# yinyunie/Pose2Room

Measured on AMD Instinct MI355X. Metric: P2RNet train-step samples/sec (T=1024,J=53,bs=32), higher is better.
Workload: dtype f32; 1 GPU; P2RNet full train step, bs=32/GPU, T=1024, J=53, seeds=512, proposals=128 (BASELINE configs[2]); input=P2RNet_dataloader over SyntheticPoseDataset, global_batch=32, frames=1024, parallelism=dp1

## Files before the change

### pose2room_amd/p2rnet/modules/stgcn.py

```python
import torch
import torch.nn as nn

from ..registers import MODULES
from .stgcn_layers import Graph, st_gcn_block
from .sub_modules import SingleConv


def _point_mlp(cin, width, cout):
    return nn.Sequential(SingleConv(cin, width, kernel_size=1, order='cbr', padding=0, ndim=1),
                         SingleConv(width, width, kernel_size=1, order='cbr', padding=0, ndim=1),
                         SingleConv(width, cout, kernel_size=1, order='c', padding=0, ndim=1))


@MODULES.register_module
class STGCN(nn.Module):
    def __init__(self, cfg, optim_spec=None):
        super().__init__()
        self.optim_spec = optim_spec

        self.graph = Graph(layout='virtualroom', strategy='spatial', max_hop=5)
        self.register_buffer('A', torch.tensor(self.graph.A, dtype=torch.float32, requires_grad=False))

        self.n_seeds = cfg.config['data']['num_seeds']
        self.origin_joint_id = cfg.dataset_config.origin_joint_id
        width, out_channels = 64, 256
        kernel_size = (3, self.A.size(0))
        self.knn = 20

        self.pos_embed = _point_mlp(3, 64, width)
        self.sk_feat = _point_mlp(3, 64, width)
        self.st_gcn_networks = nn.ModuleList(
            [st_gcn_block(width, 64, kernel_size, 1, residual=False)] +
            [st_gcn_block(64, 64, kernel_size, 1) for _ in range(5)])
        from ..gcn_op import GraphTables
        tables = GraphTables(self.graph.A)
        for i, blk in enumerate(self.st_gcn_networks):
            blk.gcn.tables = tables
            blk.chain_input = i > 0
        self.conv_joint = nn.Conv1d(cfg.dataset_config.joint_num * 64, out_channels, kernel_size=1)
        self.edge_importance = nn.ParameterList(
            [nn.Parameter(torch.ones(self.A.size())) for _ in self.st_gcn_networks])

        n_frames = cfg.config['data']['num_frames']
        if self.n_seeds >= n_frames:
            self.seed_inds = torch.round(torch.linspace(0, n_frames - 1, self.n_seeds)).long()
        else:
            self.seed_sampling = cfg.config['data']['seed_sampling']

    def _select_seeds(self, hip):
        n_batch, n_frames, _ = hip.shape
        device = hip.device
        if self.n_seeds >= n_frames:
            return self.seed_inds.repeat(n_batch, 1).to(device)
        if self.seed_sampling == 'random':
            inds = torch.argsort(torch.rand(size=(n_batch, n_frames)), dim=1)[:, :self.n_seeds]
            return torch.sort(inds, dim=1)[0].to(device)
        if self.seed_sampling == 'uniform':
            step = torch.norm(torch.diff(hip, dim=1), dim=2)
            cum = torch.cumsum(torch.cat([torch.zeros(size=(n_batch, 1), device=device), step], dim=1).double(),
                               dim=1).float()
            stride = cum[:, -1] / (self.n_seeds - 1)
            target = stride.unsqueeze(-1) * torch.arange(self.n_seeds, dtype=torch.float, device=device)
            if cum.is_cuda and cum.dtype == torch.float32 and n_frames <= 40000:
                from .. import seed_op
                return seed_op.nearest_prefix(cum, target)
            return torch.argmin(torch.abs(cum.unsqueeze(-1) - target.unsqueeze(1)), dim=1)
        raise NotImplementedError

    @staticmethod
    def _mlp(seq, x, inner, add_ct=None):
        from .. import bn_op, tconv_op, embed_op
        if embed_op.supported(seq, x, inner, add_ct):
            return embed_op.embed_mlp(seq, x, inner, add_ct)
        s0, s1, s2 = seq
        fused = (x.is_cuda and len(seq) == 3 and hasattr(s0, 'batchnorm') and hasattr(s1, 'batchnorm')
                 and not hasattr(s2, 'batchnorm') and tconv_op.supported_embed3(x, s0.conv)
                 and x.shape[2] % inner == 0 and inner <= 64)
        if fused:
            z0s = None
            if s0.batchnorm.training:
                z, z0s = tconv_op.embed3(x, s0.conv, want_stats=True)
            else:
                z = tconv_op.embed3(x, s0.conv)
            z = z.view(x.shape[0], 64, x.shape[2] // inner, inner)
            fused = tconv_op.supported_pointwise(z, s0.batchnorm, s1.conv) and \
                tconv_op.supported_pointwise(z, s1.batchnorm, s2.conv)
            if fused:
                if s1.batchnorm.training:
                    z, zs = tconv_op.bn_relu_tconv(z, s0.batchnorm, s1.conv, stats=z0s, want_stats=True)
                    z = tconv_op.bn_relu_tconv(z, s1.batchnorm, s2.conv, stats=zs, add_ct=add_ct)
                else:
                    z = tconv_op.bn_relu_tconv(z, s0.batchnorm, s1.conv)
                    z = tconv_op.bn_relu_tconv(z, s1.batchnorm, s2.conv, add_ct=add_ct)
                return z.view(x.shape[0], 64, x.shape[2])
        for stage in seq:
            if x.is_cuda and hasattr(stage, 'batchnorm') and hasattr(stage, 'ReLU') and \
                    bn_op.supported(x, stage.batchnorm):
                x = bn_op.fused_bn_act(stage.conv(x), stage.batchnorm, None, relu=True)
            else:
                x = stage(x)
        if add_ct is not None:
            x = (x.view(x.shape[0], x.shape[1], -1, inner) + add_ct.unsqueeze(-1)).view(x.shape)
        return x

    def embed(self, input_joints):
        n_batch, n_frames, n_joints, _ = input_joints.shape
        device = input_joints.device
        hip = input_joints[:, :, self.origin_joint_id]
        win = torch.arange(n_frames, device=device).unsqueeze(-1) + \
            torch.arange(-self.knn // 2, self.knn // 2, device=device).unsqueeze(0)
        win = win.clamp_(0, n_frames - 1)
        offs = hip[:, win] - hip.unsqueeze(2)
        pe = self._mlp(self.pos_embed, offs.reshape(n_batch, n_frames * self.knn, 3).transpose(1, 2).contiguous(), self.knn)
        from .. import seed_op
        pe = pe.view(n_batch, -1, n_frames, self.knn)
        fused = seed_op.short_rows_supported(pe)
        pe = seed_op.mean_last(pe) if fused else pe.mean(dim=3)
        rel = input_joints - input_joints[:, :, self.origin_joint_id:self.origin_joint_id + 1]
        sk = self._mlp(self.sk_feat, rel.reshape(n_batch, n_frames * n_joints, 3).transpose(1, 2).contiguous(), n_joints,
                       add_ct=pe)
        return sk.view(n_batch, -1, n_frames, n_joints)

    def forward(self, input_joints, end_points=None):
        end_points = {} if end_points is None else end_points
        n_batch, n_frames, n_joints, n_dim = input_joints.size()
        seed_inds = self._select_seeds(input_joints[:, :, self.origin_joint_id])

        x = self.embed(input_joints)
        blocks = self.st_gcn_networks
        tables = blocks[0].gcn.tables
        if tables is not None and tables.gen2 and all(b.chainable(x, self.A) for b in blocks):
            from ..gcn_op import prepare_chain
            for gcn, prep in zip(blocks, prepare_chain(blocks, self.A, self.edge_importance, tables, frames=x.shape[2])):
                x, _ = gcn(x, prep.Aeff, prepared=prep)
        else:
            for gcn, importance in zip(blocks, self.edge_importance):
                x, _ = gcn(x, self.A * importance)

        seed_skeleton = torch.gather(
            input_joints, 1, seed_inds[:, :, None, None].expand(n_batch, self.n_seeds, n_joints, n_dim))
        if self.n_seeds < n_frames:
            from .. import seed_op
            if seed_op.seed_rows_supported(x, seed_inds):
                rows = seed_op.seed_rows(x, seed_inds)
            else:
                rows = x.permute(0, 2, 1, 3)[torch.arange(n_batch, device=x.device)[:, None], seed_inds]
            seed_features = torch.nn.functional.linear(
                rows.reshape(n_batch, self.n_seeds, -1),
                self.conv_joint.weight.squeeze(-1), self.conv_joint.bias)
        else:
            x = x.transpose(2, 3).reshape(n_batch, -1, n_frames)
            seed_features = self.conv_joint(x).transpose(1, 2)
            seed_features = torch.gather(
                seed_features, 1, seed_inds.unsqueeze(-1).expand(n_batch, self.n_seeds, seed_features.size(-1)))
        end_points['seed_inds'] = seed_inds
        end_points['seed_skeleton'] = seed_skeleton[..., :3]
        end_points['seed_features'] = seed_features
        return end_points
```

### pose2room_amd/p2rnet/modules/stgcn_layers.py

```python
from collections import deque

import numpy as np
import torch
import torch.nn as nn

_VIRTUALROOM_BONES = [
    (0, 1), (1, 3), (3, 5), (5, 19), (0, 2), (2, 4), (4, 6), (6, 20), (0, 7), (7, 8), (8, 9),
    (9, 10), (10, 21), (10, 22), (8, 11), (11, 13), (13, 15), (15, 17), (8, 12), (12, 14),
    (14, 16), (16, 18), (17, 23), (23, 24), (24, 25), (17, 26), (26, 27), (27, 28), (17, 29),
    (29, 30), (30, 31), (17, 32), (32, 33), (33, 34), (17, 35), (35, 36), (36, 37), (18, 38),
    (38, 39), (39, 40), (18, 41), (41, 42), (42, 43), (18, 44), (44, 45), (45, 46), (18, 47),
    (47, 48), (48, 49), (18, 50), (50, 51), (51, 52)]

_LAYOUTS = {'virtualroom': dict(num_node=53, bones=_VIRTUALROOM_BONES, center=0)}


def hop_distance(num_node, edges, max_hop):
    nbr = [[] for _ in range(num_node)]
    for i, j in edges:
        if i != j:
            nbr[i].append(j)
            nbr[j].append(i)
    hop = np.full((num_node, num_node), np.inf)
    for s in range(num_node):
        hop[s, s] = 0
        dq = deque([s])
        while dq:
            u = dq.popleft()
            if hop[s, u] >= max_hop:
                continue
            for v in nbr[u]:
                if np.isinf(hop[s, v]):
                    hop[s, v] = hop[s, u] + 1
                    dq.append(v)
    return hop


class Graph:

    def __init__(self, layout='virtualroom', strategy='spatial', max_hop=5, dilation=1):
        if layout not in _LAYOUTS:
            raise ValueError("Do Not Exist This Layout.")
        spec = _LAYOUTS[layout]
        self.max_hop, self.dilation = max_hop, dilation
        self.num_node, self.center = spec['num_node'], spec['center']
        self.edge = [(i, i) for i in range(self.num_node)] + list(spec['bones'])
        self.hop_dis = hop_distance(self.num_node, self.edge, max_hop)
        self.A = self._adjacency(strategy)

    def _adjacency(self, strategy):
        V = self.num_node
        hops = list(range(0, self.max_hop + 1, self.dilation))
        reach = np.zeros((V, V))
        for h in hops:
            reach[self.hop_dis == h] = 1
        col = reach.sum(0)
        inv = np.zeros(V)
        inv[col > 0] = col[col > 0] ** (-1)
        norm = reach * inv[None, :]
        if strategy == 'uniform':
            return norm[None]
        if strategy == 'distance':
            return np.stack([np.where(self.hop_dis == h, norm, 0.0) for h in hops])
        if strategy == 'spatial':
            dc = self.hop_dis[:, self.center]
            same = dc[:, None] == dc[None, :]
            closer = dc[:, None] > dc[None, :]
            planes = []
            for h in hops:
                at_h = self.hop_dis == h
                root = np.where(at_h & same, norm, 0.0)
                close = np.where(at_h & closer, norm, 0.0)
                further = np.where(at_h & ~same & ~closer, norm, 0.0)
                if h == 0:
                    planes.append(root)
                else:
                    planes.append(root + close)
                    planes.append(further)
            return np.stack(planes)
        raise ValueError("Do Not Exist This Strategy")


class ConvTemporalGraphical(nn.Module):

    def __init__(self, in_channels, out_channels, kernel_size, t_kernel_size=1, t_stride=1,
                 t_padding=0, t_dilation=1, bias=True):
        super().__init__()
        self.kernel_size = kernel_size
        self.out_channels = out_channels
        self.tables = None
        self.fused = True
        self.conv = nn.Conv2d(in_channels, out_channels * kernel_size, kernel_size=(t_kernel_size, 1),
                              padding=(t_padding, 0), stride=(t_stride, 1), dilation=(t_dilation, 1),
                              bias=bias)

    def forward(self, x, A, want_stats=False, with_residual=False, bn_link=None, prepared=None, lazy_res=False):
        assert A.size(0) == self.kernel_size
        if self.tables is not None and self.fused:
            from .. import gcn_op
            if gcn_op.supported(x, self.conv.weight, A):
                return gcn_op.graph_conv(x, self.conv.weight, self.conv.bias, A, self.tables, want_stats,
                                         with_residual, bn_link, prepared, lazy_res), A
        assert not want_stats and not with_residual and prepared is None
        y = self.conv(x)
        n, kc, t, v = y.size()
        y = y.view(n, self.kernel_size, kc // self.kernel_size, t, v)
        z = torch.einsum('nkctv,kvw->nctw', (y, A))
        return z.contiguous(), A


def _zero(x):
    return 0


def _iden(x):
    return x


class st_gcn_block(nn.Module):

    def __init__(self, in_channels, out_channels, kernel_size, stride=1, dropout=0, residual=True):
        super().__init__()
        assert len(kernel_size) == 2 and kernel_size[0] % 2 == 1
        padding = ((kernel_size[0] - 1) // 2, 0)
        self.gcn = ConvTemporalGraphical(in_channels, out_channels, kernel_size[1])
        self.tcn = nn.Sequential(
            nn.BatchNorm2d(out_channels),
            nn.ReLU(inplace=True),
            nn.Conv2d(out_channels, out_channels, (kernel_size[0], 1), (stride, 1), padding),
            nn.BatchNorm2d(out_channels),
            nn.Dropout(dropout, inplace=True),
        )
        if not residual:
            self.residual = _zero
        elif in_channels == out_channels and stride == 1:
            self.residual = _iden
        else:
            self.residual = nn.Sequential(
                nn.Conv2d(in_channels, out_channels, kernel_size=1, stride=(stride, 1)),
                nn.BatchNorm2d(out_channels))
        self.relu = nn.ReLU(inplace=True)

    fused_bn = True
    fused_tconv = True
    lazy_residual_grad = True
    chain_input = False

    def chainable(self, x, A):
        if not (self.fused_bn and x.is_cuda and self.tcn[4].p == 0):
            return False
        from .. import bn_op, gcn_op, tconv_op
        return (self.training and self.fused_tconv and self.gcn.tables is not None and self.gcn.fused
                and gcn_op.supported(x, self.gcn.conv.weight, A) and bn_op.supported(x, self.tcn[0])
                and tconv_op.supported(x, self.tcn[0], self.tcn[2]))

    def forward(self, x, A, prepared=None):
        res = self.residual(x)
        if self.fused_bn and x.is_cuda and self.tcn[4].p == 0:
            from .. import bn_op, gcn_op, tconv_op
            chain = self.chainable(x, A)
            assert chain or prepared is None
            lazy = False
            if chain:
                if self.residual is _iden and x.requires_grad:
                    in_link = getattr(x, '_p2r_bn_link', None) if self.chain_input else None
                    lazy = self.lazy_residual_grad and self.tcn[3].training
                    (z, zstats, res), A = self.gcn(x, A, want_stats=True, with_residual=True, bn_link=in_link,
                                                   prepared=prepared, lazy_res=lazy)
                else:
                    (z, zstats), A = self.gcn(x, A, want_stats=True, prepared=prepared)
                wp = (prepared.tcn_wp_f, prepared.tcn_wp_b) if prepared is not None and z.shape[3] == 53 else None
                u, ustats = tconv_op.bn_relu_tconv(z, self.tcn[0], self.tcn[2], stats=zstats, want_stats=True, wp=wp)
                res_t = res if torch.is_tensor(res) else None
                return bn_op.fused_bn_act(u, self.tcn[3], res_t, relu=True, stats=ustats, link=bn_op.BNLink(),
                                          lazy_res=lazy), A
            x, A = self.gcn(x, A)
            if bn_op.supported(x, self.tcn[0]):
                if self.fused_tconv and tconv_op.supported(x, self.tcn[0], self.tcn[2]):
                    u = tconv_op.bn_relu_tconv(x, self.tcn[0], self.tcn[2])
                else:
                    h = bn_op.fused_bn_act(x, self.tcn[0], None, relu=True)
                    u = self.tcn[2](h)
                res_t = res if torch.is_tensor(res) else None
                return bn_op.fused_bn_act(u, self.tcn[3], res_t, relu=True), A
        else:
            x, A = self.gcn(x, A)
        x = self.tcn(x) + res
        return self.relu(x), A
```

### pose2room_amd/p2rnet/seed_op.py

```python
import torch
from torch.autograd import Function

from .. import _lib


def _rowsum(x, V, scale):
    out = torch.empty(x.shape[:-1], dtype=torch.float32, device=x.device)
    _lib.launch("p2r_rowsum_short", x.device, x.numel() // V, V, scale, x, out)
    return out


def short_rows_supported(x):
    return x.is_cuda and x.dtype == torch.float32 and 1 <= x.shape[-1] <= 64


class _SeedRows(Function):

    @staticmethod
    def forward(ctx, x, seed_inds):
        x = x.contiguous()
        inds = seed_inds.long().contiguous()
        B, C, T, J = x.shape
        S = inds.shape[1]
        out = torch.empty((B, S, C * J), dtype=torch.float32, device=x.device)
        _lib.launch("p2r_gather_frames", x.device, B, C, T, J, S, x, inds, out)
        ctx.save_for_backward(inds)
        ctx.dims = (B, C, T, J, S)
        return out

    @staticmethod
    def backward(ctx, dout):
        (inds,) = ctx.saved_tensors
        B, C, T, J, S = ctx.dims
        dout = dout.contiguous()
        dx = torch.empty((B, C, T, J), dtype=torch.float32, device=dout.device)
        _lib.launch("p2r_gather_frames_grad", dout.device, B, C, T, J, S, dout, inds, dx)
        return dx, None


def seed_rows_supported(x, seed_inds):
    return (x.is_cuda and x.dtype == torch.float32 and x.dim() == 4 and seed_inds.is_cuda and seed_inds.dim() == 2
            and seed_inds.dtype in (torch.int64, torch.int32) and seed_inds.shape[0] == x.shape[0])


def seed_rows(x, seed_inds):
    return _SeedRows.apply(x, seed_inds)


class _MeanLast(Function):

    @staticmethod
    def forward(ctx, x):
        x = x.contiguous()
        ctx.shape = x.shape
        return _rowsum(x, x.shape[-1], 1.0 / x.shape[-1])

    @staticmethod
    def backward(ctx, g):
        return (g * (1.0 / ctx.shape[-1])).unsqueeze(-1).expand(ctx.shape)


def mean_last(x):
    return _MeanLast.apply(x)


class _AddBroadcastLast(Function):

    @staticmethod
    def forward(ctx, a, b):
        ctx.V = a.shape[-1]
        return a + b.unsqueeze(-1)

    @staticmethod
    def backward(ctx, g):
        db = None
        if ctx.needs_input_grad[1]:
            gc = g.contiguous()
            db = _rowsum(gc, ctx.V, 1.0)
        return (g if ctx.needs_input_grad[0] else None), db


def add_broadcast_last(a, b):
    return _AddBroadcastLast.apply(a, b)


def nearest_prefix(cum, target):
    cum, target = cum.contiguous(), target.contiguous()
    B, T = cum.shape
    S = target.shape[1]
    out = torch.empty((B, S), dtype=torch.int64, device=cum.device)
    _lib.launch("p2r_nearest_prefix", cum.device, B, T, S, cum, target, out)
    return out
```

Baseline: 794.1 samples/s.

## Fuse last ST-GCN block's BN+ReLU+residual with seed-frame gather

In the last ST-GCN block, the final batchnorm-plus-residual-plus-ReLU is fused with the gather of seed frames, so only the S seed rows are written instead of the full B×C×T×J activation. The backward pass gets new kernels: a per-batch frame-to-seed inverse map, a reduction over seed rows for the BN gradient statistics, and an apply kernel that writes the input and residual gradients with scatter-add over duplicate seeds. This removes a full-tensor elementwise write/read and a separate gather kernel, at the cost of several new kernels and a separately built shared library.

```diff
diff --git a/include/p2r_seed_seam.h b/include/p2r_seed_seam.h
--- /dev/null
+++ b/include/p2r_seed_seam.h
@@ -0,0 +1,24 @@
+#ifndef P2R_SEED_SEAM_H
+#define P2R_SEED_SEAM_H
+
+#include "p2r_hip.h"
+
+#ifdef __cplusplus
+extern "C" {
+#endif
+
+int p2r_seed_map(int b, int t, int s, const long long *inds, int *off, int *lst, void *stream);
+int p2r_seed_rows_bn(int b, int c, int t, int j, int s, const float *z, const float *scale, const float *shift,
+                     const float *res, const long long *inds, float *rows, void *stream);
+int p2r_seed_bn_bwd_partials(int b, int s);
+int p2r_seed_bn_bwd_reduce(int b, int c, int t, int j, int s, const float *d_rows, const float *z, const float *res,
+                           const float *fin, const long long *inds, float *partial, void *stream);
+int p2r_seed_bn_bwd_apply(int b, int c, int t, int j, int s, const float *d_rows, const float *z, const float *res,
+                          const float *fin, const float *m1, const float *m2, const int *off, const int *lst, float *g,
+                          float *dres, unsigned char *mask, void *stream);
+
+#ifdef __cplusplus
+}
+#endif
+
+#endif
diff --git a/pose2room_amd/csrc/seed_seam.hip b/pose2room_amd/csrc/seed_seam.hip
--- /dev/null
+++ b/pose2room_amd/csrc/seed_seam.hip
@@ -0,0 +1,338 @@
+#include "p2r_common.h"
+#include "../../include/p2r_seed_seam.h"
+
+namespace {
+
+constexpr int SM_THREADS = 256;
+
+__global__ __launch_bounds__(SM_THREADS) void seed_map_kernel(int T, int S, const long long *__restrict__ inds,
+                                                              int *__restrict__ off, int *__restrict__ lst) {
+  extern __shared__ int sm[];
+  int *s_ind = sm, *s_lst = sm + S, *s_off = sm + 2 * S, *s_cur = s_off + T + 1, *s_part = s_cur + T;
+  const int b = blockIdx.x, tid = threadIdx.x;
+  for (int t = tid; t < T; t += SM_THREADS) s_cur[t] = 0;
+  for (int s = tid; s < S; s += SM_THREADS) {
+    const long long v = inds[(size_t)b * S + s];
+    s_ind[s] = (v >= 0 && v < T) ? (int)v : -1;
+  }
+  __syncthreads();
+  for (int s = tid; s < S; s += SM_THREADS)
+    if (s_ind[s] >= 0) atomicAdd(&s_cur[s_ind[s]], 1);
+  __syncthreads();
+  const int per = (T + SM_THREADS - 1) / SM_THREADS;
+  const int lo = min(T, tid * per), hi = min(T, lo + per);
+  int mine = 0;
+  for (int t = lo; t < hi; ++t) mine += s_cur[t];
+  s_part[tid] = mine;
+  __syncthreads();
+  for (int d = 1; d < SM_THREADS; d <<= 1) {
+    const int v = tid >= d ? s_part[tid - d] : 0;
+    __syncthreads();
+    s_part[tid] += v;
+    __syncthreads();
+  }
+  int pos = s_part[tid] - mine;
+  for (int t = lo; t < hi; ++t) {
+    const int cnt = s_cur[t];
+    s_off[t] = pos;
+    s_cur[t] = pos;
+    pos += cnt;
+  }
+  const int total = s_part[SM_THREADS - 1];
+  if (tid == 0) s_off[T] = total;
+  __syncthreads();
+  for (int s = tid; s < S; s += SM_THREADS)
+    if (s_ind[s] >= 0) s_lst[atomicAdd(&s_cur[s_ind[s]], 1)] = s;
+  __syncthreads();
+  for (int t = lo; t < hi; ++t) {
+    const int o0 = s_off[t], o1 = s_off[t + 1];
+    for (int i = o0 + 1; i < o1; ++i) {
+      const int v = s_lst[i];
+      int k = i - 1;
+      for (; k >= o0 && s_lst[k] > v; --k) s_lst[k + 1] = s_lst[k];
+      s_lst[k + 1] = v;
+    }
+  }
+  __syncthreads();
+  int *ob = off + (size_t)b * (T + 1), *lb = lst + (size_t)b * S;
+  for (int t = tid; t <= T; t += SM_THREADS) ob[t] = s_off[t];
+  for (int i = tid; i < S; i += SM_THREADS) lb[i] = i < total ? s_lst[i] : -1;
+}
+
+__global__ __launch_bounds__(256) void seed_rows_bn_kernel(int C, int T, int J, int S, const float *__restrict__ z,
+                                                           const float *__restrict__ scale,
+                                                           const float *__restrict__ shift,
+                                                           const float *__restrict__ res,
+                                                           const long long *__restrict__ inds,
+                                                           float *__restrict__ rows) {
+  const int b = blockIdx.x / S;
+  const long long t = inds[blockIdx.x];
+  const int lane = threadIdx.x & 63, wave = threadIdx.x >> 6;
+  float *o = rows + (size_t)blockIdx.x * C * J;
+  if (t < 0 || t >= T) {
+    for (int e = threadIdx.x; e < C * J; e += 256) o[e] = 0.f;
+    return;
+  }
+  const size_t fb = ((size_t)b * C * T + t) * J, cs = (size_t)T * J;
+  for (int j = lane; j < J; j += 64) {
+    int c = wave;
+    for (; c + 28 < C; c += 32) {
+      float v[8], r[8];
+#pragma unroll
+      for (int u = 0; u < 8; ++u) {
+        v[u] = __builtin_nontemporal_load(z + fb + (size_t)(c + 4 * u) * cs + j);
+        r[u] = res ? __builtin_nontemporal_load(res + fb + (size_t)(c + 4 * u) * cs + j) : 0.f;
+      }
+#pragma unroll
+      for (int u = 0; u < 8; ++u) {
+        const float y = fmaf(v[u], scale[c + 4 * u], shift[c + 4 * u]) + r[u];
+        o[(c + 4 * u) * J + j] = fmaxf(y, 0.f);
+      }
+    }
+    for (; c < C; c += 4) {
+      const float y = fmaf(z[fb + (size_t)c * cs + j], scale[c], shift[c]) + (res ? res[fb + (size_t)c * cs + j] : 0.f);
+      o[c * J + j] = fmaxf(y, 0.f);
+    }
+  }
+}
+
+constexpr int SR_SEEDS = 8;
+
+__global__ __launch_bounds__(256) void seed_bn_bwd_reduce_kernel(int C, int T, int J, int S, int groups,
+                                                                 const float *__restrict__ d_rows,
+                                                                 const float *__restrict__ z,
+                                                                 const float *__restrict__ res,
+                                                                 const float *__restrict__ fin,
+                                                                 const long long *__restrict__ inds,
+                                                                 float2 *__restrict__ partial) {
+  const int b = blockIdx.x / groups, s0 = (blockIdx.x - b * groups) * SR_SEEDS;
+  const int lane = threadIdx.x & 63, wave = threadIdx.x >> 6;
+  int fr[SR_SEEDS];
+#pragma unroll
+  for (int u = 0; u < SR_SEEDS; ++u) {
+    const long long t = s0 + u < S ? inds[(size_t)b * S + s0 + u] : -1;
+    fr[u] = (t >= 0 && t < T) ? (int)t : -1;
+  }
+  const size_t cs = (size_t)T * J, n = (size_t)C * J;
+  for (int c = wave; c < C; c += 4) {
+    const float mu = fin[c], is = fin[C + c], sc = fin[2 * C + c], sh = fin[3 * C + c];
+    const size_t zb = ((size_t)b * C + c) * cs;
+    float sg = 0.f, sq = 0.f;
+    for (int j = lane; j < J; j += 64) {
+      float g[SR_SEEDS], zv[SR_SEEDS], rv[SR_SEEDS];
+#pragma unroll
+      for (int u = 0; u < SR_SEEDS; ++u) {
+        const bool on = fr[u] >= 0;
+        const size_t zi = zb + (size_t)(on ? fr[u] : 0) * J + j;
+        g[u] = on ? d_rows[((size_t)b * S + s0 + u) * n + (size_t)c * J + j] : 0.f;
+        zv[u] = on ? z[zi] : 0.f;
+        rv[u] = (on && res) ? res[zi] : 0.f;
+      }
+#pragma unroll
+      for (int u = 0; u < SR_SEEDS; ++u) {
+        const float gm = (fmaf(zv[u], sc, sh) + rv[u]) > 0.f ? g[u] : 0.f;
+        sg += gm;
+        sq += gm * ((zv[u] - mu) * is);
+      }
+    }
+#pragma unroll
+    for (int o = 32; o >= 1; o >>= 1) { sg += __shfl_xor(sg, o, 64); sq += __shfl_xor(sq, o, 64); }
+    if (lane == 0) partial[(size_t)blockIdx.x * C + c] = make_float2(sg, sq);
+  }
+}
+
+constexpr int SA_TT = 8, SA_THREADS = 448;
+typedef float f4s __attribute__((ext_vector_type(4)));
+
+__global__ __launch_bounds__(SA_THREADS) void seed_bn_bwd_apply_kernel(int C, int T, int J, int S,
+                                                                       const float *__restrict__ d_rows,
+                                                                       const float *__restrict__ z,
+                                                                       const float *__restrict__ res,
+                                                                       const float *__restrict__ fin,
+                                                                       const float *__restrict__ m1,
+                                                                       const float *__restrict__ m2,
+                                                                       const int *__restrict__ off,
+                                                                       const int *__restrict__ lst,
+                                                                       float *__restrict__ g,
+                                                                       float *__restrict__ dres,
+                                                                       unsigned char *__restrict__ mask) {
+  const int chunks = (T + SA_TT - 1) / SA_TT;
+  const int b = blockIdx.x / chunks, t0 = (blockIdx.x - b * chunks) * SA_TT;
+  const size_t n = (size_t)C * J, cs = (size_t)T * J;
+  const int *ob = off + (size_t)b * (T + 1), *lb = lst + (size_t)b * S;
+  for (int e = threadIdx.x; e < SA_TT * J; e += SA_THREADS) {
+    const int f = e / J, j = e - f * J;
+    if (t0 + f >= T) continue;
+    const int o0 = ob[t0 + f], cnt = ob[t0 + f + 1] - o0;
+    const size_t xb = ((size_t)b * C * T + t0) * J + e;
+    const float *r0 = d_rows + ((size_t)b * S + (cnt > 0 ? lb[o0] : 0)) * n + j;
+    const float *r1 = d_rows + ((size_t)b * S + (cnt > 1 ? lb[o0 + 1] : 0)) * n + j;
+    int c = 0;
+    for (; c + 8 <= C; c += 8) {
+      float zv[8], rv[8], a[8];
+#pragma unroll
+      for (int u = 0; u < 8; ++u) {
+        zv[u] = z[xb + (size_t)(c + u) * cs];
+        rv[u] = (cnt > 0 && res) ? res[xb + (size_t)(c + u) * cs] : 0.f;
+        a[u] = cnt > 0 ? r0[(c + u) * J] : 0.f;
+        if (cnt > 1) a[u] += r1[(c + u) * J];
+      }
+      if (cnt > 2)
+        for (int i = 2; i < cnt; ++i) {
+          const float *ri = d_rows + ((size_t)b * S + lb[o0 + i]) * n + j;
+#pragma unroll
+          for (int u = 0; u < 8; ++u) a[u] += ri[(c + u) * J];
+        }
+#pragma unroll
+      for (int u = 0; u < 8; ++u) {
+        const int cc = c + u;
+        const bool open = cnt > 0 && (fmaf(zv[u], fin[2 * C + cc], fin[3 * C + cc]) + rv[u]) > 0.f;
+        const float gm = open ? a[u] : 0.f;
+        const float xh = (zv[u] - fin[cc]) * fin[C + cc];
+        g[xb + (size_t)cc * cs] = fin[2 * C + cc] * (gm - m1[cc] - xh * m2[cc]);
+        if (dres) dres[xb + (size_t)cc * cs] = gm;
+        if (mask) mask[xb + (size_t)cc * cs] = open;
+      }
+    }
+    for (; c < C; ++c) {
+      const float zv = z[xb + (size_t)c * cs];
+      float a = 0.f;
+      for (int i = 0; i < cnt; ++i) a += d_rows[((size_t)b * S + lb[o0 + i]) * n + (size_t)c * J + j];
+      const float rv = (cnt > 0 && res) ? res[xb + (size_t)c * cs] : 0.f;
+      const bool open = cnt > 0 && (fmaf(zv, fin[2 * C + c], fin[3 * C + c]) + rv) > 0.f;
+      const float gm = open ? a : 0.f;
+      const float xh = (zv - fin[c]) * fin[C + c];
+      g[xb + (size_t)c * cs] = fin[2 * C + c] * (gm - m1[c] - xh * m2[c]);
+      if (dres) dres[xb + (size_t)c * cs] = gm;
+      if (mask) mask[xb + (size_t)c * cs] = open;
+    }
+  }
+}
+
+__global__ __launch_bounds__(256) void seed_bn_bwd_apply4_kernel(int C, int T, int J, int S,
+                                                                 const float *__restrict__ d_rows,
+                                                                 const float *__restrict__ z,
+                                                                 const float *__restrict__ res,
+                                                                 const float *__restrict__ fin,
+                                                                 const float *__restrict__ m1,
+                                                                 const float *__restrict__ m2,
+                                                                 const int *__restrict__ off,
+                                                                 const int *__restrict__ lst,
+                                                                 float *__restrict__ g,
+                                                                 float *__restrict__ dres,
+                                                                 unsigned char *__restrict__ mask) {
+  const int chunks = (T + SA_TT - 1) / SA_TT;
+  const int b = blockIdx.x / chunks, t0 = (blockIdx.x - b * chunks) * SA_TT;
+  const int nq = min(SA_TT, T - t0) * J / 4;
+  const int q = threadIdx.x & 127, half = threadIdx.x >> 7;
+  if (q >= nq) return;
+  const size_t n = (size_t)C * J, cs = (size_t)T * J;
+  const int *ob = off + (size_t)b * (T + 1), *lb = lst + (size_t)b * S;
+  int cnt[4], o0[4];
+  const float *r0[4], *r1[4];
+  const float *db = d_rows + (size_t)b * S * n;
+#pragma unroll
+  for (int i = 0; i < 4; ++i) {
+    const int e = 4 * q + i, f = e / J, j = e - f * J;
+    o0[i] = ob[t0 + f];
+    cnt[i] = ob[t0 + f + 1] - o0[i];
+    r0[i] = db + (size_t)(cnt[i] > 0 ? lb[o0[i]] : 0) * n + j;
+    r1[i] = db + (size_t)(cnt[i] > 1 ? lb[o0[i] + 1] : 0) * n + j;
+  }
+  const bool any = (cnt[0] | cnt[1] | cnt[2] | cnt[3]) != 0;
+  const bool more = cnt[0] > 2 || cnt[1] > 2 || cnt[2] > 2 || cnt[3] > 2;
+  const size_t xb = ((size_t)b * C * T + t0) * J + 4 * (size_t)q;
+#pragma unroll 4
+  for (int c = half; c < C; c += 2) {
+    const size_t xi = xb + (size_t)c * cs;
+    const f4s zv4 = __builtin_nontemporal_load(reinterpret_cast<const f4s *>(z + xi));
+    f4s rv4 = {0.f, 0.f, 0.f, 0.f};
+    if (any && res) rv4 = __builtin_nontemporal_load(reinterpret_cast<const f4s *>(res + xi));
+    float a[4];
+#pragma unroll
+    for (int i = 0; i < 4; ++i) {
+      a[i] = cnt[i] > 0 ? r0[i][c * J] : 0.f;
+      if (cnt[i] > 1) a[i] += r1[i][c * J];
+    }
+    if (more)
+#pragma unroll
+      for (int i = 0; i < 4; ++i)
+        for (int k = 2; k < cnt[i]; ++k) {
+          const int e = 4 * q + i, j = e - (e / J) * J;
+          a[i] += db[(size_t)lb[o0[i] + k] * n + (size_t)c * J + j];
+        }
+    const float mu = fin[c], is = fin[C + c], sc = fin[2 * C + c], sh = fin[3 * C + c], a1 = m1[c], a2 = m2[c];
+    f4s go, ro;
+    unsigned mk = 0;
+#pragma unroll
+    for (int i = 0; i < 4; ++i) {
+      const bool open = cnt[i] > 0 && (fmaf(zv4[i], sc, sh) + rv4[i]) > 0.f;
+      const float gm = open ? a[i] : 0.f;
+      const float xh = (zv4[i] - mu) * is;
+      go[i] = sc * (gm - a1 - xh * a2);
+      ro[i] = gm;
+      mk |= (open ? 1u : 0u) << (8 * i);
+    }
+    __builtin_nontemporal_store(go, reinterpret_cast<f4s *>(g + xi));
+    if (dres) __builtin_nontemporal_store(ro, reinterpret_cast<f4s *>(dres + xi));
+    if (mask) __builtin_nontemporal_store(mk, reinterpret_cast<unsigned *>(mask + xi));
+  }
+}
+
+}
+
+extern "C" int p2r_seed_map(int b, int t, int s, const long long *inds, int *off, int *lst, void *stream) {
+  if (b < 0 || t <= 0 || s <= 0 || 2LL * s + 2LL * t + 1 + SM_THREADS > 16384) return P2R_EINVAL;
+  if (b == 0) return P2R_OK;
+  const size_t lds = (2 * (size_t)s + 2 * (size_t)t + 1 + SM_THREADS) * sizeof(int);
+  hipLaunchKernelGGL(seed_map_kernel, dim3((unsigned)b), dim3(SM_THREADS), lds, p2r_stream(stream), t, s, inds, off, lst);
+  P2R_LAUNCH_CHECK();
+  return P2R_OK;
+}
+
+extern "C" int p2r_seed_rows_bn(int b, int c, int t, int j, int s, const float *z, const float *scale, const float *shift,
+                                const float *res, const long long *inds, float *rows, void *stream) {
+  if (b < 0 || c <= 0 || t <= 0 || j <= 0 || s < 0) return P2R_EINVAL;
+  if (b == 0 || s == 0) return P2R_OK;
+  hipLaunchKernelGGL(seed_rows_bn_kernel, dim3((unsigned)(b * s)), dim3(256), 0, p2r_stream(stream), c, t, j, s, z, scale,
+                     shift, res, inds, rows);
+  P2R_LAUNCH_CHECK();
+  return P2R_OK;
+}
+
+extern "C" int p2r_seed_bn_bwd_partials(int b, int s) {
+  if (b < 0 || s <= 0) return 0;
+  return b * ((s + SR_SEEDS - 1) / SR_SEEDS);
+}
+
+extern "C" int p2r_seed_bn_bwd_reduce(int b, int c, int t, int j, int s, const float *d_rows, const float *z,
+                                      const float *res, const float *fin, const long long *inds, float *partial,
+                                      void *stream) {
+  if (b < 0 || c <= 0 || t <= 0 || j <= 0 || s <= 0) return P2R_EINVAL;
+  if (b == 0) return P2R_OK;
+  const int groups = (s + SR_SEEDS - 1) / SR_SEEDS;
+  hipLaunchKernelGGL(seed_bn_bwd_reduce_kernel, dim3((unsigned)(b * groups)), dim3(256), 0, p2r_stream(stream), c, t, j, s,
+                     groups, d_rows, z, res, fin, inds, reinterpret_cast<float2 *>(partial));
+  P2R_LAUNCH_CHECK();
+  return P2R_OK;
+}
+
+extern "C" int p2r_seed_bn_bwd_apply(int b, int c, int t, int j, int s, const float *d_rows, const float *z,
+                                     const float *res, const float *fin, const float *m1, const float *m2, const int *off,
+                                     const int *lst, float *g, float *dres, unsigned char *mask, void *stream) {
+  if (b < 0 || c <= 0 || t <= 0 || j <= 0 || s <= 0) return P2R_EINVAL;
+  if (b == 0) return P2R_OK;
+  const dim3 grid((unsigned)(b * ((t + SA_TT - 1) / SA_TT)));
+  const bool vec = j <= 64 && ((long long)t * j) % 4 == 0 && (uintptr_t)mask % 4 == 0 &&
+                   ((uintptr_t)z | (uintptr_t)res | (uintptr_t)g | (uintptr_t)dres) % 16 == 0;
+  if (vec) {
+    hipLaunchKernelGGL(seed_bn_bwd_apply4_kernel, grid, dim3(256), 0, p2r_stream(stream), c, t, j, s, d_rows, z, res, fin, m1,
+                       m2, off, lst, g, dres, mask);
+    P2R_LAUNCH_CHECK();
+    return P2R_OK;
+  }
+  hipLaunchKernelGGL(seed_bn_bwd_apply_kernel, grid, dim3(SA_THREADS), 0, p2r_stream(stream), c, t, j, s, d_rows, z, res,
+                     fin, m1, m2, off, lst, g, dres, mask);
+  P2R_LAUNCH_CHECK();
+  return P2R_OK;
+}
diff --git a/pose2room_amd/p2rnet/modules/stgcn.py b/pose2room_amd/p2rnet/modules/stgcn.py
--- a/pose2room_amd/p2rnet/modules/stgcn.py
+++ b/pose2room_amd/p2rnet/modules/stgcn.py
@@ -131,9 +131,16 @@
         tables = blocks[0].gcn.tables
         if tables is not None and tables.gen2 and all(b.chainable(x, self.A) for b in blocks):
             from ..gcn_op import prepare_chain
-            for gcn, prep in zip(blocks, prepare_chain(blocks, self.A, self.edge_importance, tables, frames=x.shape[2])):
-                x, _ = gcn(x, prep.Aeff, prepared=prep)
+            from .. import bn_op, math_mode, seed_op
+            seam = (self.n_seeds < n_frames and bn_op.GATE_HOOK is None and not math_mode.split16()
+                    and seed_op.seed_rows_bn_supported(x, blocks[-1].tcn[3], seed_inds))
+            for i, (gcn, prep) in enumerate(zip(blocks, prepare_chain(blocks, self.A, self.edge_importance, tables,
+                                                                      frames=x.shape[2]))):
+                last = seam and i == len(blocks) - 1
+                x, _ = gcn(x, prep.Aeff, prepared=prep, seed_inds=seed_inds if last else None)
+            rows = x if seam else None
         else:
+            rows = None
             for gcn, importance in zip(blocks, self.edge_importance):
                 x, _ = gcn(x, self.A * importance)
 
@@ -141,7 +148,9 @@
             input_joints, 1, seed_inds[:, :, None, None].expand(n_batch, self.n_seeds, n_joints, n_dim))
         if self.n_seeds < n_frames:
             from .. import seed_op
-            if seed_op.seed_rows_supported(x, seed_inds):
+            if rows is not None:
+                x = None
+            elif seed_op.seed_rows_supported(x, seed_inds):
                 rows = seed_op.seed_rows(x, seed_inds)
             else:
                 rows = x.permute(0, 2, 1, 3)[torch.arange(n_batch, device=x.device)[:, None], seed_inds]
diff --git a/pose2room_amd/p2rnet/modules/stgcn_layers.py b/pose2room_amd/p2rnet/modules/stgcn_layers.py
--- a/pose2room_amd/p2rnet/modules/stgcn_layers.py
+++ b/pose2room_amd/p2rnet/modules/stgcn_layers.py
@@ -154,12 +154,12 @@
                 and gcn_op.supported(x, self.gcn.conv.weight, A) and bn_op.supported(x, self.tcn[0])
                 and tconv_op.supported(x, self.tcn[0], self.tcn[2]))
 
-    def forward(self, x, A, prepared=None):
+    def forward(self, x, A, prepared=None, seed_inds=None):
         res = self.residual(x)
         if self.fused_bn and x.is_cuda and self.tcn[4].p == 0:
             from .. import bn_op, gcn_op, tconv_op
             chain = self.chainable(x, A)
-            assert chain or prepared is None
+            assert chain or (prepared is None and seed_inds is None)
             lazy = False
             if chain:
                 if self.residual is _iden and x.requires_grad:
@@ -172,6 +172,9 @@
                 wp = (prepared.tcn_wp_f, prepared.tcn_wp_b) if prepared is not None and z.shape[3] == 53 else None
                 u, ustats = tconv_op.bn_relu_tconv(z, self.tcn[0], self.tcn[2], stats=zstats, want_stats=True, wp=wp)
                 res_t = res if torch.is_tensor(res) else None
+                if seed_inds is not None:
+                    from .. import seed_op
+                    return seed_op.seed_rows_bn(u, self.tcn[3], res_t, ustats, seed_inds, lazy_res=lazy), A
                 return bn_op.fused_bn_act(u, self.tcn[3], res_t, relu=True, stats=ustats, link=bn_op.BNLink(),
                                           lazy_res=lazy), A
             x, A = self.gcn(x, A)
diff --git a/pose2room_amd/p2rnet/seed_op.py b/pose2room_amd/p2rnet/seed_op.py
--- a/pose2room_amd/p2rnet/seed_op.py
+++ b/pose2room_amd/p2rnet/seed_op.py
@@ -1,7 +1,34 @@
+import ctypes
+import os
+
 import torch
 from torch.autograd import Function
 
 from .. import _lib
+
+SEAM_HEADER_PATH = os.path.join(os.path.dirname(_lib.HEADER_PATH), "p2r_seed_seam.h")
+SEAM_LIB_PATH = os.path.join(os.path.dirname(os.path.abspath(_lib.__file__)), "libp2r_seed_seam.so")
+_seam_lib = None
+
+
+def seam_lib():
+    global _seam_lib
+    if _seam_lib is None:
+        if not os.path.exists(SEAM_LIB_PATH):
+            raise _lib.P2RLibraryError(f"{SEAM_LIB_PATH} is missing: build it with `make -C pose2room_amd/csrc` "
+                                       "(pose2room_amd has no CPU fallback)")
+        l = ctypes.CDLL(SEAM_LIB_PATH)
+        for name, proto in _lib.prototypes(SEAM_HEADER_PATH).items():
+            fn = getattr(l, name)
+            fn.restype, fn.argtypes = proto.restype, proto.argtypes
+        _seam_lib = l
+    return _seam_lib
+
+
+def _seam_launch(name, device, *args):
+    fn = getattr(seam_lib(), name)
+    with torch.cuda.device(device):
+        _lib.check(fn(*[a.data_ptr() if torch.is_tensor(a) else a for a in args], _lib.current_stream(device)), name)
 
 
 def _rowsum(x, V, scale):
@@ -45,6 +72,60 @@
 
 def seed_rows(x, seed_inds):
     return _SeedRows.apply(x, seed_inds)
+
+
+class _SeedRowsBN(Function):
+
+    @staticmethod
+    def forward(ctx, z, weight, bias, res, fin, seed_inds, lazy_res=False):
+        z = z.contiguous()
+        res_c = res.contiguous() if res is not None else None
+        inds = seed_inds.long().contiguous()
+        B, C, T, J = z.shape
+        S = inds.shape[1]
+        rows = torch.empty((B, S, C * J), dtype=torch.float32, device=z.device)
+        _seam_launch("p2r_seed_rows_bn", z.device, B, C, T, J, S, z, fin[2], fin[3], res_c, inds, rows)
+        ctx.save_for_backward(z, res_c, fin, inds)
+        ctx.lazy_res = bool(lazy_res) and res is not None
+        return rows
+
+    @staticmethod
+    def backward(ctx, d_rows):
+        from . import bn_op, handoff
+        z, res, fin, inds = ctx.saved_tensors
+        B, C, T, J = z.shape
+        S = inds.shape[1]
+        dev = z.device
+        d_rows = d_rows.contiguous()
+        off = torch.empty((B, T + 1), dtype=torch.int32, device=dev)
+        lst = torch.empty((B, S), dtype=torch.int32, device=dev)
+        _seam_launch("p2r_seed_map", dev, B, T, S, inds, off, lst)
+        part = torch.empty((seam_lib().p2r_seed_bn_bwd_partials(B, S), C, 2), dtype=torch.float32, device=dev)
+        _seam_launch("p2r_seed_bn_bwd_reduce", dev, B, C, T, J, S, d_rows, z, res, fin, inds, part)
+        tot = bn_op.bwd_finalize(part, B * T * J)
+        g = torch.empty_like(z)
+        dres = torch.empty_like(z) if (res is not None and ctx.needs_input_grad[3]) else None
+        mask = torch.empty(z.shape, dtype=torch.uint8, device=dev) if (dres is not None and ctx.lazy_res) else None
+        _seam_launch("p2r_seed_bn_bwd_apply", dev, B, C, T, J, S, d_rows, z, res, fin, tot[2], tot[3], off, lst, g, dres, mask)
+        if mask is not None:
+            handoff.put(dres, 'res_mask', mask)
+        return g, tot[1], tot[0], dres, None, None, None
+
+
+SEED_ROWS_BN = True
+
+
+def seed_rows_bn_supported(z, bn, seed_inds):
+    from . import bn_op
+    return (SEED_ROWS_BN and seed_rows_supported(z, seed_inds) and bn.training and bn_op.supported(z, bn) and z.shape[0] > 0
+            and 0 < seed_inds.shape[1] < z.shape[2] and seed_inds.shape[1] + z.shape[2] <= 8063)
+
+
+def seed_rows_bn(z, bn, res, stats, seed_inds, lazy_res=False):
+    from . import bn_op
+    part = bn_op._stats_partial(z.contiguous()) if stats is None else stats
+    fin = bn_op.finalize(part, z.numel() // z.shape[1], bn)
+    return _SeedRowsBN.apply(z, bn.weight, bn.bias, res, fin, seed_inds, lazy_res)
 
 
 class _MeanLast(Function):
```

Result: no change. 797.0 samples/s, median of 6 (+0.4%).
